# cfframe/spatial-VAE

Hardware: AMD Instinct MI355X
Metric: images/sec (ELBO fwd+bwd+step), MNIST 28x28 batch=256, 1/2/4/8 GPU (higher is better)
Workload: dtype f32; 1 GPU; mnist-rotated-translated 28x28 z=2 H=500x2 tanh B=256 (BASELINE configs[1]); global_batch=256, per_gpu_batch=256, pixels=784, parallelism=dp1

## Files before the change

spatial_vae_amd/csrc/dense.h:

```cpp
#pragma once
#include "common.h"

namespace svae {

struct DenseArgs {
    const float* in;
    const float* wp;
    float* out;
    const float* bias;
    const float* aux;
    long tiles;
    int Hp;
    int H;
    int act;
    int resid;
    PoseArgs pose;
    const float4* posebuf;
    const float* tab;
    float* sgtile;
    float* dfpart;
    long Mp;
    int N, Timg;
    const float* do_p;
    const float* out_w;
// ... 605 lines not shown
#pragma unroll
        for (int t = 0; t < 4; ++t) {
            xa[t] = *reinterpret_cast<const float4*>(sl + t * 256);
            xb[t] = *reinterpret_cast<const float4*>(sl + (4 + t) * 256);
        }
        d = *reinterpret_cast<const float4*>(ring + ((o - o0) & 3) * kSlotFloats + 8 * 256 + h * 4);
    };
    auto frag_post = [&](long o, float4 (&xa)[4], const float4& d) {
        if (own_out) {
            const float wgt = (o < o1) ? 1.0f : 0.0f;
            pbias[0] += wgt * ((d.x + d.y) + (d.z + d.w));
#pragma unroll
            for (int t = 0; t < 4; ++t) pw[0][t] += wgt * ((d.x * xa[t].x + d.y * xa[t].y) + (d.z * xa[t].z + d.w * xa[t].w));
        }
#pragma unroll
        for (int t = 0; t < 4; ++t) {
            const float4 v = xa[t];
            const float4 tt = make_float4(d.x * v.x, d.y * v.y, d.z * v.z, d.w * v.w);
            xa[t] = make_float4(__builtin_fmaf(-tt.x, v.x, R1 == 1 ? d.x : tt.x), __builtin_fmaf(-tt.y, v.y, R1 == 1 ? d.y : tt.y),
                                __builtin_fmaf(-tt.z, v.z, R1 == 1 ? d.z : tt.z), __builtin_fmaf(-tt.w, v.w, R1 == 1 ? d.w : tt.w));
        }
    };
    auto mul = [&](const float4 (&xa)[4], const float4 (&xb)[4]) {
#pragma unroll
        for (int i = 0; i < 4; ++i)
#pragma unroll
            for (int j = 0; j < 4; ++j) acc[i][j] = __builtin_amdgcn_mfma_f32_32x32x2f32(xa[i].x, xb[j].x, acc[i][j], 0, 0, 0);
#pragma unroll
        for (int i = 0; i < 4; ++i)
#pragma unroll
            for (int j = 0; j < 4; ++j) acc[i][j] = __builtin_amdgcn_mfma_f32_32x32x2f32(xa[i].y, xb[j].y, acc[i][j], 0, 0, 0);
#pragma unroll
        for (int i = 0; i < 4; ++i)
#pragma unroll
            for (int j = 0; j < 4; ++j) acc[i][j] = __builtin_amdgcn_mfma_f32_32x32x2f32(xa[i].z, xb[j].z, acc[i][j], 0, 0, 0);
#pragma unroll
        for (int i = 0; i < 4; ++i)
#pragma unroll
            for (int j = 0; j < 4; ++j) acc[i][j] = __builtin_amdgcn_mfma_f32_32x32x2f32(xa[i].w, xb[j].w, acc[i][j], 0, 0, 0);
        if (own_bias) {
#pragma unroll
            for (int t = 0; t < 4; ++t) bs[t] += (xa[t].x + xa[t].y) + (xa[t].z + xa[t].w);
        }
    };
    if (o0 < o1) {
        float4 ca[4], cb[4], na[4], nb[4];
        dma(o0);
        dma(o0 + 1);
        dma(o0 + 2);
        if (CL > 0) asm volatile("s_waitcnt vmcnt(18)" ::: "memory");
        else asm volatile("s_waitcnt vmcnt(16)" ::: "memory");
        float4 nd = make_float4(0.f, 0.f, 0.f, 0.f);
        if (R1 != 0) {
            frag_raw(o0, ca, cb, nd);
            frag_post(o0, ca, nd);
        } else {
            frag(o0, ca, cb);
        }
        for (long o = o0; o < o1; ++o) {
            dma(o + 3);
            if (CL > 0) asm volatile("s_waitcnt vmcnt(18)" ::: "memory");
            else asm volatile("s_waitcnt vmcnt(16)" ::: "memory");
            if (R1 != 0) frag_raw(o + 1, na, nb, nd);
            else frag(o + 1, na, nb);
            if (CL == 0 || R1 != 0) __builtin_amdgcn_sched_barrier(0);
            mul(ca, cb);
            if (CL == 0 || R1 != 0) __builtin_amdgcn_sched_barrier(0);
            if (R1 != 0) frag_post(o + 1, na, nd);
#pragma unroll
            for (int t = 0; t < 4; ++t) {
                ca[t] = na[t];
                cb[t] = nb[t];
            }
        }
        dma_wait_all();
    }

    float* slab = a.slab + (long)split * Hp * Hp;
#pragma unroll
    for (int i = 0; i < 4; ++i) {
        if (ibase + i >= ntile) continue;
#pragma unroll
        for (int j = 0; j < 4; ++j) {
            if (jbase + j >= ntile) continue;
            const int k = (jbase + j) * 32 + nl;
#pragma unroll
            for (int r = 0; r < 16; ++r) {
                const int n = (ibase + i) * 32 + (r & 3) + 8 * (r >> 2) + 4 * h;
                slab[(long)n * Hp + k] = acc[i][j][r];
            }
        }
    }
    if (own_out) {
#pragma unroll
        for (int c = 0; c < CL; ++c) {
#pragma unroll
            for (int i = 0; i < 4; ++i)
                if (ibase + i < ntile) a.wpart[(((long)split * 2 + h) * CL + c) * Hp + (ibase + i) * 32 + nl] = pw[c][i];
            if (bi == 0 && wave == 0 && nl == 0) a.bpart[((long)split * 2 + h) * CL + c] = pbias[c];
        }
    }
    if (own_bias) {
#pragma unroll
        for (int i = 0; i < 4; ++i)
            if (ibase + i < ntile) a.bslab[((long)split * 2 + h) * Hp + (ibase + i) * 32 + nl] = bs[i];
    }
}

struct WgradReduceArgs {
    const float* slab;
    const float* bslab;
    float* dW;
    float* db;
    int H, Hp, S;
    const float* row_scale;
};
__device__ __forceinline__ void wgrad_reduce_block(const WgradReduceArgs& a, unsigned bx, float (*red)[64]) {
    const float* __restrict__ slab = a.slab;
    const float* __restrict__ bslab = a.bslab;
    float* __restrict__ dW = a.dW;
    float* __restrict__ db = a.db;
    const float* __restrict__ row_scale = a.row_scale;
    const int H = a.H, Hp = a.Hp, S = a.S;
    const int col = threadIdx.x & 63, grp = threadIdx.x >> 6;
    const long idx = (long)bx * 64 + col;
    const bool in = idx < (long)H * H;
    float part = 0.0f;
    if (in) {
        const int n = (int)(idx / H), k = (int)(idx - (long)n * H);
        const float* p = slab + (long)n * Hp + k;
        const long st = (long)Hp * Hp;
        float s0 = 0.0f, s1 = 0.0f, s2 = 0.0f, s3 = 0.0f;
        int i = grp;
        for (; i + 12 < S; i += 16) {
            s0 += p[(long)i * st];
            s1 += p[(long)(i + 4) * st];
            s2 += p[(long)(i + 8) * st];
            s3 += p[(long)(i + 12) * st];
        }
        for (; i < S; i += 4) s0 += p[(long)i * st];
        part = (s0 + s1) + (s2 + s3);
    }
    red[grp][col] = part;
    __syncthreads();
    if (grp == 0 && in && dW) {
        const float t = (red[0][col] + red[1][col]) + (red[2][col] + red[3][col]);
        dW[idx] = row_scale ? t * row_scale[idx / H] : t;
    }
    if (db && bx * 64 < (unsigned)H) {
        __syncthreads();
        const int n = bx * 64 + col;
        float s = 0.0f;
        if (n < H)
            for (int i = grp; i < 2 * S; i += 4) s += bslab[(long)i * Hp + n];
        red[grp][col] = s;
        __syncthreads();
        if (grp == 0 && n < H) {
            const float t = (red[0][col] + red[1][col]) + (red[2][col] + red[3][col]);
            db[n] = row_scale ? t * row_scale[n] : t;
        }
    }
}
__global__ void __launch_bounds__(256) wgrad_reduce_kernel(WgradReduceArgs a) {
    __shared__ float red[4][64];
    wgrad_reduce_block(a, blockIdx.x, red);
}

}
```

spatial_vae_amd/csrc/elementwise.h:

```cpp
#pragma once
#include <type_traits>
#include "common.h"

namespace svae {

__device__ __forceinline__ long slab_index(int contr, int out, int ntile) {
    return (((long)(contr >> 3) * ntile + (out >> 5)) * 2 + ((contr >> 2) & 1)) * 128 + (out & 31) * 4 + (contr & 3);
}
struct PrepareArgs {
    const float* coord_w; const float* coord_b; const float* latent_w; const float* bil_w; const float* z;
    float* tab; float4* posebuf; PoseArgs pose;
    int B, H, Hp, Zd, in_dim;
    int nb_tab, nb_pack, nlayers;
    const float* W[SVAE_MAX_HIDDEN]; float* wf[SVAE_MAX_HIDDEN]; float* wb[SVAE_MAX_HIDDEN];
    const float* wb_row_scale[SVAE_MAX_HIDDEN];
};
__global__ void __launch_bounds__(256) prepare_kernel(PrepareArgs a) {
    if ((int)blockIdx.x < a.nb_tab) {
        const long idx = (long)blockIdx.x * 256 + threadIdx.x;
        if (idx < a.B) {
            float c, s, d0, d1;
            image_pose(a.pose, (int)idx, c, s, d0, d1);
            a.posebuf[idx] = make_float4(c, s, d0, d1);
        }
        if (idx >= (long)a.B * a.Hp) return;
        const int b = idx / a.Hp, k = idx % a.Hp;
        float out[kSlots] = {0, 0, 0, 0, 0, 0, 0, 0};
        if (k < a.H) {
            for (int p = 0; p < a.in_dim; ++p) {
                float w = a.coord_w[k * a.in_dim + p];
                if (a.bil_w)
                    for (int q = 0; q < a.Zd; ++q) w += a.bil_w[((long)k * a.in_dim + p) * a.Zd + q] * a.z[(long)b * a.Zd + q];
                out[p] = w;
            }
            float bias = a.coord_b[k];
            if (a.latent_w)
                for (int q = 0; q < a.Zd; ++q) bias += a.latent_w[(long)k * a.Zd + q] * a.z[(long)b * a.Zd + q];
            out[kBiasSlot] = bias;
        }
        float4* dst = reinterpret_cast<float4*>(a.tab + idx * kSlots);
        dst[0] = make_float4(out[0], out[1], out[2], out[3]);
        dst[1] = make_float4(out[4], out[5], out[6], out[7]);
        return;
    }
    const int rel = blockIdx.x - a.nb_tab;
    const int l = rel / a.nb_pack;
    const long idx = (long)(rel - l * a.nb_pack) * 256 + threadIdx.x;
    if (l >= a.nlayers || idx >= (long)a.Hp * a.Hp) return;
    const int n = idx / a.Hp, k = idx % a.Hp;
    const float v = (n < a.H && k < a.H) ? a.W[l][(long)n * a.H + k] : 0.0f;
    a.wf[l][slab_index(k, n, a.Hp / 32)] = v;
    a.wb[l][slab_index(n, k, a.Hp / 32)] = (a.wb_row_scale[l] && n < a.H) ? v * a.wb_row_scale[l][n] : v;
}

struct RowGeo {
    int N, Npad, Hp, in_dim, act, B;
};

constexpr int kL0Chunk = 32;
template <int ACT>
__global__ void __launch_bounds__(256) layer0_fwd_kernel(PoseArgs pose, const float4* __restrict__ posebuf,
                                                         const float* __restrict__ tab, float* __restrict__ a0, RowGeo g,
                                                         int oct_per_chunk, int chunks_per_image, long nchunks) {
    __shared__ float4 xs[kL0Chunk * 2 * 2];
    const long chunk = (long)blockIdx.z * gridDim.y + blockIdx.y;
    if (chunk >= nchunks) return;
    const int b = (int)(chunk / chunks_per_image), ci = (int)(chunk - (long)b * chunks_per_image);
    const int oimg = g.Npad >> 3;
    const int oc0 = ci * oct_per_chunk;
    const int noc = (oc0 + oct_per_chunk <= oimg) ? oct_per_chunk : oimg - oc0;
    const float4 pb = posebuf[b];
    const float* cbase = pose.coords ? pose.coords + (long)b * g.N * 2 : pose.grid;
    float* xf = reinterpret_cast<float*>(xs);
    for (int j = threadIdx.x; j < noc * 8; j += 256) {
        const int i = oc0 * 8 + j;
        float x0 = 0.0f, x1 = 0.0f;
        if (i < g.N) {
            const float2 raw = *reinterpret_cast<const float2*>(cbase + (long)i * 2);
            x0 = pb.x * raw.x - pb.y * raw.y + pb.z;
            x1 = pb.y * raw.x + pb.x * raw.y + pb.w;
        }
        const int slot = (j >> 2) * 8 + (j & 3);
        xf[slot] = x0;
        xf[slot + 4] = x1;
    }
    __syncthreads();
    const int t = blockIdx.x * 256 + threadIdx.x;
    if (t >= g.Hp * 2) return;
    const int h = t & 1, k = t >> 1;
    const float4* tp = reinterpret_cast<const float4*>(tab + ((long)b * g.Hp + k) * kSlots);
    const float4 t0 = tp[0], t1 = tp[1];
    const long ostride = (long)g.Hp * 8;
    float* dst = a0 + (((long)b * oimg + oc0) * g.Hp * 2 + t) * 4;
    const bool expand = g.in_dim == 5;
#pragma unroll 4
    for (int jo = 0; jo < noc; ++jo) {
        const float4 X0 = xs[(jo * 2 + h) * 2], X1 = xs[(jo * 2 + h) * 2 + 1];
        const float x0[4] = {X0.x, X0.y, X0.z, X0.w}, x1[4] = {X1.x, X1.y, X1.z, X1.w};
        float out[4];
#pragma unroll
        for (int e = 0; e < 4; ++e) {
            float v = t1.y + x0[e] * t0.x + x1[e] * t0.y;
            if (expand) v += (x0[e] * x0[e]) * t0.z + (x1[e] * x1[e]) * t0.w + (x0[e] * x1[e]) * t1.x;
            out[e] = act_fwd<ACT>(v);
        }
        *reinterpret_cast<float4*>(dst + jo * ostride) = make_float4(out[0], out[1], out[2], out[3]);
    }
}

template <int C>
__global__ void out_fwd_kernel(const float* __restrict__ a, const float* __restrict__ out_w,
                               const float* __restrict__ out_b, float* __restrict__ y, float* __restrict__ logits,
                               RowGeo g, int H, int softplus, long noct) {
    const int lane = threadIdx.x & 63;
    const int nl = lane & 31, h = lane >> 5;
    const long wave0 = (long)blockIdx.x * 4 + (threadIdx.x >> 6);
    const long nwaves = (long)gridDim.x * 4;
    for (long o = wave0; o < noct; o += nwaves) {
        float p[4][C];
#pragma unroll
        for (int e = 0; e < 4; ++e)
#pragma unroll
            for (int c = 0; c < C; ++c) p[e][c] = 0.0f;
        for (int t = 0; t < g.Hp / 32; ++t) {
            const int n = t * 32 + nl;
            const float4 v = *reinterpret_cast<const float4*>(a + ((o * g.Hp + n) * 8 + 4 * h));
#pragma unroll
            for (int c = 0; c < C; ++c) {
                const float w = (n < H) ? out_w[c * H + n] : 0.0f;
                p[0][c] += v.x * w; p[1][c] += v.y * w; p[2][c] += v.z * w; p[3][c] += v.w * w;
            }
        }
#pragma unroll
        for (int e = 0; e < 4; ++e)
#pragma unroll
            for (int c = 0; c < C; ++c) p[e][c] = wave_sum32(p[e][c]);
        if (nl < 4) {
            const long m = 8 * o + 4 * h + nl;
            const int b = m / g.Npad, i = m % g.Npad;
            if (i < g.N) {
#pragma unroll
                for (int c = 0; c < C; ++c) {
                    const float s0 = nl == 0 ? p[0][c] : nl == 1 ? p[1][c] : nl == 2 ? p[2][c] : p[3][c];
                    const float lg = s0 + out_b[c];
                    float s = 1.0f / (1.0f + expf(-lg));
                    if (softplus && c == 0) s = log1pf(expf(s));
                    const long oi = ((long)b * g.N + i) * C + c;
                    y[oi] = s;
                    if (logits) logits[oi] = lg;
                }
            }
        }
    }
}

__global__ void logits_finish_kernel(const float* __restrict__ lpart, const float* __restrict__ out_b, float* __restrict__ y,
                                     float* __restrict__ logits, RowGeo g, int C, int nblk, int softplus, long Mp, long m_split,
                                     int nblk_tail) {
    const long t = (long)blockIdx.x * 256 + threadIdx.x;
    if (t >= (long)g.B * g.N) return;
    const int b = (int)(t / g.N), i = (int)(t - (long)b * g.N);
    const long m = (long)b * g.Npad + i;
    if (m >= m_split) nblk = nblk_tail;
    for (int c = 0; c < C; ++c) {
        float lg = 0.0f;
        for (int k = 0; k < nblk; ++k) lg += lpart[((long)k * C + c) * Mp + m];
        lg += out_b[c];
        float s = 1.0f / (1.0f + expf(-lg));
        if (softplus && c == 0) s = log1pf(expf(s));
        y[t * C + c] = s;
        if (logits) logits[t * C + c] = lg;
    }
}

__global__ void __launch_bounds__(1024) logits_finish_bce_kernel(const float* __restrict__ lpart, const float* __restrict__ out_b,
                                                                const float* __restrict__ target, float* __restrict__ y,
                                                                float* __restrict__ logits, float* __restrict__ loglik,
                                                                float* __restrict__ dll, RowGeo g, int C, int nblk, long Mp,
                                                                long m_split, int nblk_tail) {
    __shared__ float red[16];
    const int b = blockIdx.x;
    float acc = 0.0f;
    const int per = (g.N + gridDim.y - 1) / gridDim.y;
    const int i0 = blockIdx.y * per, i1 = (i0 + per < g.N) ? i0 + per : g.N;
    for (int i = i0 + threadIdx.x; i < i1; i += blockDim.x) {
        const long m = (long)b * g.Npad + i;
        const long t = (long)b * g.N + i;
        const int nbk = m >= m_split ? nblk_tail : nblk;
        for (int c = 0; c < C; ++c) {
            float lg = 0.0f;
            for (int k = 0; k < nbk; ++k) lg += lpart[((long)k * C + c) * Mp + m];
            lg += out_b[c];
            const float s = 1.0f / (1.0f + expf(-lg));
            const float tg = target[t * C + c];
            y[t * C + c] = s;
            if (logits) logits[t * C + c] = lg;
            const float ls = fmaxf(logf(s), -100.0f);
            const float l1s = fmaxf(log1pf(-s), -100.0f);
            acc += tg * ls + (1.0f - tg) * l1s;
            if (dll) dll[t * C + c] = -(s - tg) / fmaxf((1.0f - s) * s, 1e-12f);
        }
    }
    acc = block_sum_waves(acc, red);
    if (threadIdx.x == 0) loglik[(long)b * gridDim.y + blockIdx.y] = acc;
}

__global__ void loglik_reduce_kernel(const float* __restrict__ part, float* __restrict__ loglik, int B, int chunks) {
    const int b = blockIdx.x * 256 + threadIdx.x;
    if (b >= B) return;
    float s = 0.0f;
    for (int k = 0; k < chunks; ++k) s += part[(long)b * chunks + k];
    loglik[b] = s;
}

__global__ void dlogits_kernel(const float* __restrict__ logits, const float* __restrict__ dy,
                               const float* __restrict__ dy_scale, float* __restrict__ do_p, int B, int N, int Npad,
                               int C, int softplus, long Mp, unsigned* __restrict__ amax) {
    const long idx = (long)blockIdx.x * 256 + threadIdx.x;
    float m = 0.0f;
    if (idx < (long)C * Mp) {
        const int c = (int)(idx / Mp);
        const long mp = idx - (long)c * Mp;
        const int b = (int)(mp / Npad), i = (int)(mp - (long)b * Npad);
        float v = 0.0f;
        if (i < N) {
            const long src = ((long)b * N + i) * C + c;
            const float lg = logits[src];
            const float s = 1.0f / (1.0f + expf(-lg));
            float g = dy[src];
            if (dy_scale) g *= dy_scale[b];
            if (softplus && c == 0) g *= 1.0f / (1.0f + expf(-s));
            v = g * s * (1.0f - s);
        }
        do_p[idx] = v;
        m = fabsf(v);
    }
    if (amax) {
        __shared__ float red[4];
#pragma unroll
        for (int d = 32; d >= 1; d >>= 1) m = fmaxf(m, __shfl_xor(m, d));
        if ((threadIdx.x & 63) == 0) red[threadIdx.x >> 6] = m;
        __syncthreads();
        if (threadIdx.x == 0) {
            m = fmaxf(fmaxf(red[0], red[1]), fmaxf(red[2], red[3]));
            if (m > 0.0f) atomicMax(amax, __float_as_uint(m));
        }
    }
}

template <int ACT, int C>
__global__ void out_bwd_kernel(const float* __restrict__ a, const float* __restrict__ do_p,
                               const float* __restrict__ out_w, float* __restrict__ dh, float* __restrict__ wpart,
                               float* __restrict__ bpart, int H, int Hp, long Mp, long noct, long oct_per_chunk) {
    const int t = blockIdx.x * 256 + threadIdx.x;
    if (t >= Hp * 2) return;
    const int h = t & 1, n = t >> 1;
    float w[C], pw[C], pb[C];
#pragma unroll
    for (int c = 0; c < C; ++c) {
        w[c] = (n < H) ? out_w[c * H + n] : 0.0f;
        pw[c] = 0.0f;
        pb[c] = 0.0f;
    }
    const long o0 = blockIdx.y * oct_per_chunk;
    const long o1 = (o0 + oct_per_chunk < noct) ? o0 + oct_per_chunk : noct;
    for (long o = o0; o < o1; ++o) {
        const long off = (o * Hp + n) * 8 + 4 * h;
        const float4 av = *reinterpret_cast<const float4*>(a + off);
        float4 da = make_float4(0.f, 0.f, 0.f, 0.f);
#pragma unroll
        for (int c = 0; c < C; ++c) {
            const float4 d = *reinterpret_cast<const float4*>(do_p + (long)c * Mp + 8 * o + 4 * h);
            da.x += d.x * w[c]; da.y += d.y * w[c]; da.z += d.z * w[c]; da.w += d.w * w[c];
            pw[c] += (d.x * av.x + d.y * av.y) + (d.z * av.z + d.w * av.w);
            pb[c] += (d.x + d.y) + (d.z + d.w);
        }
        da.x *= act_grad<ACT>(av.x); da.y *= act_grad<ACT>(av.y);
        da.z *= act_grad<ACT>(av.z); da.w *= act_grad<ACT>(av.w);
        *reinterpret_cast<float4*>(dh + off) = da;
    }
#pragma unroll
    for (int c = 0; c < C; ++c) wpart[(((long)blockIdx.y * 2 + h) * C + c) * Hp + n] = pw[c];
    if (n == 0) {
#pragma unroll
        for (int c = 0; c < C; ++c) bpart[((long)blockIdx.y * 2 + h) * C + c] = pb[c];
    }
}

constexpr int kObrLanes = 16;
struct OutBwdReduceArgs {
    const float* wpart;
    const float* bpart;
    float* dWo;
    float* dbo;
    int C, H, Hp, nparts;
};
template <int LPT>
__device__ __forceinline__ void out_bwd_reduce_block(const OutBwdReduceArgs& a, unsigned bx, float (*red)[65]) {
    static_assert(kObrLanes % LPT == 0, "whole part lanes per thread");
    constexpr int LSTEP = kObrLanes / LPT;
    const float* __restrict__ wpart = a.wpart;
    const float* __restrict__ bpart = a.bpart;
    const int C = a.C, H = a.H, Hp = a.Hp, nparts = a.nparts;
    const int col = threadIdx.x & 63, pl0 = threadIdx.x >> 6;
    const int blocks_per_c = (Hp + 63) / 64;
    if (bx == (unsigned)(C * blocks_per_c)) {
#pragma unroll
        for (int l = 0; l < LPT; ++l) {
            const int pl = pl0 + LSTEP * l;
            float s = 0.0f;
            if (col < C)
                for (int i = pl; i < nparts; i += kObrLanes) s += bpart[(long)i * C + col];
            red[pl][col] = s;
        }
        __syncthreads();
        if (pl0 == 0 && col < C && a.dbo) {
            float t = red[0][col];
#pragma unroll
            for (int j = 1; j < kObrLanes; ++j) t += red[j][col];
            a.dbo[col] = t;
        }
        return;
    }
    const int c = bx / blocks_per_c, n = (bx % blocks_per_c) * 64 + col;
    float s[LPT];
#pragma unroll
    for (int l = 0; l < LPT; ++l) s[l] = 0.0f;
    if (n < Hp) {
        const float* p = wpart + (long)c * Hp + n;
        const long st = (long)C * Hp;
        float ch[LPT][8];
        int i[LPT];
#pragma unroll
        for (int l = 0; l < LPT; ++l) {
            i[l] = pl0 + LSTEP * l;
#pragma unroll
            for (int j = 0; j < 8; ++j) ch[l][j] = 0.0f;
        }
        for (bool any = true; any;) {
            any = false;
#pragma unroll
            for (int l = 0; l < LPT; ++l)
                if (i[l] + 7 * kObrLanes < nparts) {
#pragma unroll
                    for (int j = 0; j < 8; ++j) ch[l][j] += p[(long)(i[l] + j * kObrLanes) * st];
                    i[l] += 8 * kObrLanes;
                    any = true;
                }
        }
#pragma unroll
        for (int l = 0; l < LPT; ++l) {
            for (; i[l] < nparts; i[l] += kObrLanes) ch[l][0] += p[(long)i[l] * st];
            s[l] = ((ch[l][0] + ch[l][1]) + (ch[l][2] + ch[l][3])) + ((ch[l][4] + ch[l][5]) + (ch[l][6] + ch[l][7]));
        }
    }
#pragma unroll
    for (int l = 0; l < LPT; ++l) red[pl0 + LSTEP * l][col] = s[l];
    __syncthreads();
    if (pl0 == 0 && n < H && a.dWo) {
        float t = red[0][col];
#pragma unroll
        for (int j = 1; j < kObrLanes; ++j) t += red[j][col];
        a.dWo[(long)c * H + n] = t;
    }
}
__global__ void __launch_bounds__(1024) out_bwd_reduce_kernel(const float* __restrict__ wpart, const float* __restrict__ bpart,
                                                              float* __restrict__ dWo, float* __restrict__ dbo, int C, int H,
                                                              int Hp, int nparts) {
    __shared__ float red[kObrLanes][65];
    out_bwd_reduce_block<1>(OutBwdReduceArgs{wpart, bpart, dWo, dbo, C, H, Hp, nparts}, blockIdx.x, red);
}

__global__ void layer0_bwd_params_kernel(PoseArgs pose, const float4* __restrict__ posebuf,
                                         const float* __restrict__ dh0, float* __restrict__ sgpart, RowGeo g,
                                         int oct_per_chunk, int chunks_per_image) {
    const int t = blockIdx.x * 256 + threadIdx.x;
    if (t >= g.Hp * 2) return;
    const int h = t & 1, k = t >> 1;
    const int b = blockIdx.y / chunks_per_image, ci = blockIdx.y % chunks_per_image;
    const int oimg = g.Npad / 8;
    const int oc0 = ci * oct_per_chunk;
    const int oc1 = (oc0 + oct_per_chunk < oimg) ? oc0 + oct_per_chunk : oimg;
    const float4 pb = posebuf[b];
    float G[5] = {0, 0, 0, 0, 0};
    float S = 0.0f;
    for (int oc = oc0; oc < oc1; ++oc) {
        const long o = (long)b * oimg + oc;
        const float4 d = *reinterpret_cast<const float4*>(dh0 + (o * g.Hp + k) * 8 + 4 * h);
        const float dv[4] = {d.x, d.y, d.z, d.w};
        const int i0 = oc * 8 + 4 * h;
#pragma unroll
        for (int e = 0; e < 4; ++e) {
            const float2 x = row_coord(pose, pb, b, i0 + e, g.N);
            S += dv[e];
            G[0] += dv[e] * x.x;
            G[1] += dv[e] * x.y;
            if (g.in_dim == 5) {
                G[2] += dv[e] * x.x * x.x;
                G[3] += dv[e] * x.y * x.y;
                G[4] += dv[e] * x.x * x.y;
            }
        }
    }
    float4* dst = reinterpret_cast<float4*>(sgpart + (((long)blockIdx.y * g.Hp + k) * 2 + h) * kSlots);
    dst[0] = make_float4(G[0], G[1], G[2], G[3]);
    dst[1] = make_float4(G[4], S, 0.0f, 0.0f);
}

__global__ void sg_reduce_kernel(const float* __restrict__ sgpart, float* __restrict__ sgimg, int B, int Hp,
                                 int chunks_per_image) {
    const long idx = (long)blockIdx.x * 256 + threadIdx.x;
    if (idx >= (long)B * Hp * kSlots) return;
    const int slot = idx % kSlots;
    const long bk = idx / kSlots;
    const int k = bk % Hp, b = bk / Hp;
    float s = 0.0f;
    for (int ci = 0; ci < chunks_per_image; ++ci)
        for (int h = 0; h < 2; ++h)
            s += sgpart[((((long)b * chunks_per_image + ci) * Hp + k) * 2 + h) * kSlots + slot];
    sgimg[idx] = s;
}

__global__ void layer0_bwd_coords_kernel(PoseArgs pose, const float4* __restrict__ posebuf,
                                         const float* __restrict__ dh0, const float* __restrict__ tab,
                                         float* __restrict__ dcoords, RowGeo g, long noct) {
    const int lane = threadIdx.x & 63;
    const int ml = lane & 7, kq = lane >> 3;
    const long wave0 = (long)blockIdx.x * 4 + (threadIdx.x >> 6);
    const long nwaves = (long)gridDim.x * 4;
    for (long o = wave0; o < noct; o += nwaves) {
        const long m = 8 * o + ml;
        const int b = m / g.Npad, i = m % g.Npad;
        float acc[5] = {0, 0, 0, 0, 0};
        for (int k = kq; k < g.Hp; k += 8) {
            const float d = dh0[(o * g.Hp + k) * 8 + ml];
            const float4* tp = reinterpret_cast<const float4*>(tab + ((long)b * g.Hp + k) * kSlots);
            const float4 t0 = tp[0];
            acc[0] += d * t0.x;
            acc[1] += d * t0.y;
            if (g.in_dim == 5) {
                const float4 t1 = tp[1];
                acc[2] += d * t0.z;
                acc[3] += d * t0.w;
                acc[4] += d * t1.x;
            }
        }
#pragma unroll
        for (int p = 0; p < 5; ++p) {
            acc[p] += __shfl_xor(acc[p], 8);
            acc[p] += __shfl_xor(acc[p], 16);
            acc[p] += __shfl_xor(acc[p], 32);
        }
        if (kq == 0 && i < g.N) {
            float d0 = acc[0], d1 = acc[1];
            if (g.in_dim == 5) {
                const float2 x = row_coord(pose, posebuf[b], b, i, g.N);
                d0 += 2.0f * x.x * acc[2] + x.y * acc[4];
                d1 += 2.0f * x.y * acc[3] + x.x * acc[4];
            }
            *reinterpret_cast<float2*>(dcoords + ((long)b * g.N + i) * 2) = make_float2(d0, d1);
        }
    }
}

struct FirstLayerImageArgs {
    const float* sgtile;
    int nhalf, Timg, H, Hp;
    float* sgimg;
    const float* latent_w;
    const float* bil_w;
    float* dz;
    int Zd, in_dim;
    const float* dfpart;
    int nblocks, N, Npad;
    long Mp;
    float* dcoords;
    const float* grid;
    const float4* posebuf;
    float* dtheta;
    float* ddx;
    long m_split;
    int nblocks_tail;
    const float* tab;
};
__device__ __forceinline__ void first_layer_image_block(const FirstLayerImageArgs& a, int b, int role, float* red) {
    const float* __restrict__ sgtile = a.sgtile;
    const int nhalf = a.nhalf, Timg = a.Timg, H = a.H, Hp = a.Hp;
    float* __restrict__ sgimg = a.sgimg;
    const float* __restrict__ latent_w = a.latent_w;
    const float* __restrict__ bil_w = a.bil_w;
    float* __restrict__ dz = a.dz;
    const int Zd = a.Zd, in_dim = a.in_dim;
    const float* __restrict__ dfpart = a.dfpart;
    const int nblocks = a.nblocks, N = a.N, Npad = a.Npad;
    const long Mp = a.Mp;
    float* __restrict__ dcoords = a.dcoords;
    const float* __restrict__ grid = a.grid;
    const float4* __restrict__ posebuf = a.posebuf;
    float* __restrict__ dtheta = a.dtheta;
    float* __restrict__ ddx = a.ddx;
    const long m_split = a.m_split;
    const int nblocks_tail = a.nblocks_tail;

    if (role == 0) {
        const bool pose_sums = a.tab && (dtheta || ddx);
        double pt = 0.0, p0 = 0.0, p1 = 0.0;
        float4 pb = make_float4(1.0f, 0.0f, 0.0f, 0.0f);
        if (pose_sums) pb = posebuf[b];
        for (int k = threadIdx.x; k < Hp; k += 256) {
            const float* src = sgtile + ((long)b * Timg * nhalf * Hp + k) * 4;
            const long rst = (long)Hp * 4;
            const int rows = Timg * nhalf;
            float c0[8] = {0, 0, 0, 0, 0, 0, 0, 0}, c1[8] = {0, 0, 0, 0, 0, 0, 0, 0}, c2[8] = {0, 0, 0, 0, 0, 0, 0, 0};
            double d0 = 0.0, d1 = 0.0, d2 = 0.0;
            int r = 0;
            for (; r + 7 < rows; r += 8) {
#pragma unroll
                for (int j = 0; j < 8; ++j) {
                    const float4 v = *reinterpret_cast<const float4*>(src + (r + j) * rst);
                    c0[j] += v.x; c1[j] += v.y; c2[j] += v.z;
                    if (pose_sums) { d0 += (double)v.x; d1 += (double)v.y; d2 += (double)v.z; }
                }
            }
            for (int j = 0; r < rows; ++r, ++j) {
                const float4 v = *reinterpret_cast<const float4*>(src + r * rst);
                c0[j] += v.x; c1[j] += v.y; c2[j] += v.z;
                if (pose_sums) { d0 += (double)v.x; d1 += (double)v.y; d2 += (double)v.z; }
            }
            if (pose_sums && k < H) {
                const float2 w = *reinterpret_cast<const float2*>(a.tab + ((long)b * Hp + k) * kSlots);
                p0 += (double)w.x * d2;
                p1 += (double)w.y * d2;
                pt += (double)w.y * (d0 - (double)pb.z * d2) - (double)w.x * (d1 - (double)pb.w * d2);
            }
            const float g0 = ((c0[0] + c0[1]) + (c0[2] + c0[3])) + ((c0[4] + c0[5]) + (c0[6] + c0[7]));
            const float g1 = ((c1[0] + c1[1]) + (c1[2] + c1[3])) + ((c1[4] + c1[5]) + (c1[6] + c1[7]));
            const float sv = ((c2[0] + c2[1]) + (c2[2] + c2[3])) + ((c2[4] + c2[5]) + (c2[6] + c2[7]));
            float4* dst = reinterpret_cast<float4*>(sgimg + ((long)b * Hp + k) * kSlots);
            dst[0] = make_float4(g0, g1, 0.0f, 0.0f);
            dst[1] = make_float4(0.0f, sv, 0.0f, 0.0f);
        }
        if (pose_sums) {
            double* redd = reinterpret_cast<double*>(red);
            pt = block_sum256d(pt, redd);
            p0 = block_sum256d(p0, redd);
            p1 = block_sum256d(p1, redd);
            if (threadIdx.x == 0) {
                if (dtheta) dtheta[b] = (float)pt;
                if (ddx) {
                    ddx[2 * b] = (float)p0;
                    ddx[2 * b + 1] = (float)p1;
                }
            }
        }
        if (!dz || Zd <= 0) return;
        for (int q = 0; q < Zd; ++q) {
            float s = 0.0f;
            for (int k = threadIdx.x; k < H; k += 256) {
                const float* e = sgimg + ((long)b * Hp + k) * kSlots;
                s += e[kBiasSlot] * latent_w[(long)k * Zd + q];
                if (bil_w)
                    for (int p = 0; p < in_dim; ++p) s += e[p] * bil_w[((long)k * in_dim + p) * Zd + q];
            }
            s = block_sum256(s, red);
            if (threadIdx.x == 0) dz[(long)b * Zd + q] = s;
        }
        return;
    }
    if (!dcoords) return;
    const bool want_pose = dtheta || ddx;
    float4 pb = make_float4(1.0f, 0.0f, 0.0f, 0.0f);
    if (want_pose) pb = posebuf[b];
    float st = 0.0f, s0 = 0.0f, s1 = 0.0f;
    for (int i = threadIdx.x; i < N; i += 256) {
        const long mp = (long)b * Npad + i;
        float d0 = 0.0f, d1 = 0.0f;
        const int nbk = mp >= m_split ? nblocks_tail : nblocks;
        for (int nb = 0; nb < nbk; ++nb) {
            const float2 v = *reinterpret_cast<const float2*>(dfpart + ((long)nb * Mp + mp) * 2);
            d0 += v.x; d1 += v.y;
        }
        *reinterpret_cast<float2*>(dcoords + ((long)b * N + i) * 2) = make_float2(d0, d1);
        if (want_pose) {
            const float2 gr = *reinterpret_cast<const float2*>(grid + (long)i * 2);
            st += d0 * (-pb.y * gr.x - pb.x * gr.y) + d1 * (pb.x * gr.x - pb.y * gr.y);
            s0 += d0;
            s1 += d1;
        }
    }
    if (!want_pose) return;
    st = block_sum256(st, red);
    s0 = block_sum256(s0, red);
    s1 = block_sum256(s1, red);
    if (threadIdx.x == 0) {
        if (dtheta) dtheta[b] = st;
        if (ddx) {
            ddx[2 * b] = s0;
            ddx[2 * b + 1] = s1;
        }
    }
}

__global__ void __launch_bounds__(256) first_layer_image_kernel(FirstLayerImageArgs a) {
    __shared__ __attribute__((aligned(8))) float red[8];
    first_layer_image_block(a, blockIdx.x, blockIdx.y, red);
}
__global__ void __launch_bounds__(256) backward_tail_kernel(FirstLayerImageArgs f, WgradReduceArgs r, OutBwdReduceArgs o,
                                                            unsigned nimg, unsigned nred, int B) {
    __shared__ __attribute__((aligned(8))) float red[kObrLanes * 65];
    if (blockIdx.x < nimg) first_layer_image_block(f, (int)(blockIdx.x % (unsigned)B), (int)(blockIdx.x / (unsigned)B), red);
    else if (blockIdx.x < nimg + nred) wgrad_reduce_block(r, blockIdx.x - nimg, reinterpret_cast<float (*)[64]>(red));
    else out_bwd_reduce_block<4>(o, blockIdx.x - nimg - nred, reinterpret_cast<float (*)[65]>(red));
}

constexpr int kZChunk = 8;
constexpr int kPgCols = 16, kPgLanes = 16;
__global__ void __launch_bounds__(256) layer0_param_grads_kernel(const float* __restrict__ sgimg, const float* __restrict__ z,
                                                                 float* __restrict__ dWc, float* __restrict__ dbc,
                                                                 float* __restrict__ dWz, float* __restrict__ dWbi, int B, int H,
                                                                 int Hp, int Zd, int in_dim) {
    __shared__ float red[kPgLanes][kPgCols + 1];
    const int col = threadIdx.x & (kPgCols - 1), bl = threadIdx.x / kPgCols;
    const int t = blockIdx.x * kPgCols + col;
    const bool in_range = t < H * kSlots;
    const int k = in_range ? t / kSlots : 0, slot = in_range ? t % kSlots : 0;
    const bool is_g = in_range && slot < in_dim, is_s = in_range && slot == kBiasSlot;
    const float* src = sgimg + (long)k * kSlots + slot;
    const long bstride = (long)Hp * kSlots;
    auto combine = [&](float v) {
        __syncthreads();
        red[bl][col] = v;
        __syncthreads();
        float r = red[0][col];
#pragma unroll
        for (int j = 1; j < kPgLanes; ++j) r += red[j][col];
        return r;
    };
    const bool want_z = (is_s && dWz) || (is_g && dWbi);
    const int nq0 = Zd < kZChunk ? Zd : kZChunk;
    float plain = 0.0f;
    float acc[kZChunk];
#pragma unroll
    for (int q = 0; q < kZChunk; ++q) acc[q] = 0.0f;
    if (is_g || is_s) {
        int b = bl;
        for (; b + 3 * kPgLanes < B; b += 4 * kPgLanes) {
            float v[4];
#pragma unroll
            for (int j = 0; j < 4; ++j) v[j] = src[(long)(b + j * kPgLanes) * bstride];
#pragma unroll
            for (int j = 0; j < 4; ++j) {
                plain += v[j];
                if (want_z) {
#pragma unroll
                    for (int q = 0; q < kZChunk; ++q)
                        if (q < nq0) acc[q] += v[j] * z[(long)(b + j * kPgLanes) * Zd + q];
                }
            }
        }
        for (; b < B; b += kPgLanes) {
            const float v = src[(long)b * bstride];
            plain += v;
            if (want_z) {
#pragma unroll
                for (int q = 0; q < kZChunk; ++q)
                    if (q < nq0) acc[q] += v * z[(long)b * Zd + q];
            }
        }
    }
    plain = combine(plain);
    if (bl == 0) {
        if (is_g && dWc) dWc[k * in_dim + slot] = plain;
        if (is_s && dbc) dbc[k] = plain;
    }
    for (int q0 = 0; q0 < Zd; q0 += kZChunk) {
        if (q0 > 0) {
#pragma unroll
            for (int q = 0; q < kZChunk; ++q) acc[q] = 0.0f;
            if (want_z)
                for (int b = bl; b < B; b += kPgLanes) {
                    const float v = src[(long)b * bstride];
#pragma unroll
                    for (int q = 0; q < kZChunk; ++q)
                        if (q0 + q < Zd) acc[q] += v * z[(long)b * Zd + q0 + q];
                }
        }
#pragma unroll
        for (int q = 0; q < kZChunk; ++q) {
            if (q0 + q >= Zd) break;
            const float r = combine(acc[q]);
            if (bl == 0 && want_z) {
                if (is_s) dWz[(long)k * Zd + q0 + q] = r;
                else dWbi[((long)k * in_dim + slot) * Zd + q0 + q] = r;
            }
        }
    }
}

__global__ void dz_kernel(const float* __restrict__ sgimg, const float* __restrict__ latent_w,
                          const float* __restrict__ bil_w, float* __restrict__ dz, int H, int Hp, int Zd, int in_dim) {
    __shared__ float red[4];
    const int b = blockIdx.x;
    for (int q = 0; q < Zd; ++q) {
        float s = 0.0f;
        for (int k = threadIdx.x; k < H; k += 256) {
            const float* e = sgimg + ((long)b * Hp + k) * kSlots;
            s += e[kBiasSlot] * latent_w[(long)k * Zd + q];
            if (bil_w)
                for (int p = 0; p < in_dim; ++p) s += e[p] * bil_w[((long)k * in_dim + p) * Zd + q];
        }
        s = block_sum256(s, red);
        if (threadIdx.x == 0) dz[(long)b * Zd + q] = s;
    }
}

__global__ void pose_bwd_kernel(const float* __restrict__ dcoords, const float* __restrict__ grid,
                                const float4* __restrict__ posebuf, float* __restrict__ dtheta,
                                float* __restrict__ ddx, int N) {
    __shared__ float red[4];
    const int b = blockIdx.x;
    const float4 pb = posebuf[b];
    float st = 0.0f, s0 = 0.0f, s1 = 0.0f;
    for (int i = threadIdx.x; i < N; i += 256) {
        const float2 d = *reinterpret_cast<const float2*>(dcoords + ((long)b * N + i) * 2);
        const float2 gr = *reinterpret_cast<const float2*>(grid + (long)i * 2);
        st += d.x * (-pb.y * gr.x - pb.x * gr.y) + d.y * (pb.x * gr.x - pb.y * gr.y);
        s0 += d.x;
        s1 += d.y;
    }
    st = block_sum256(st, red);
    s0 = block_sum256(s0, red);
    s1 = block_sum256(s1, red);
    if (threadIdx.x == 0) {
        if (dtheta) dtheta[b] = st;
        if (ddx) {
            ddx[2 * b] = s0;
            ddx[2 * b + 1] = s1;
        }
    }
}

__global__ void bce_kernel(const float* __restrict__ y_hat, const float* __restrict__ target,
                           float* __restrict__ loglik, float* __restrict__ dll, int n) {
    __shared__ float red[4];
    const int b = blockIdx.x;
    float acc = 0.0f;
    for (int j = threadIdx.x; j < n; j += 256) {
        const long idx = (long)b * n + j;
        const float s = y_hat[idx], t = target[idx];
        const float ls = fmaxf(logf(s), -100.0f);
        const float l1s = fmaxf(log1pf(-s), -100.0f);
        acc += t * ls + (1.0f - t) * l1s;
        if (dll) dll[idx] = -(s - t) / fmaxf((1.0f - s) * s, 1e-12f);
    }
    acc = block_sum256(acc, red);
    if (threadIdx.x == 0) loglik[b] = acc;
}

__global__ void gaussian_kernel(const float* __restrict__ yp, const float* __restrict__ target,
                                const uint8_t* __restrict__ mask, const float* __restrict__ ctf, int k,
                                float* __restrict__ loglik, float* __restrict__ dll, float* __restrict__ filt,
                                float* __restrict__ dflt, int N, int C) {
    __shared__ float red[4];
    const int b = blockIdx.x;
    const int n = (int)(sqrtf((float)N) + 0.5f);
    const float* row = yp + (long)b * N * C;
    const bool noise = C > 1;
    const int pad = k / 2;
// ... 679 lines not shown
```

spatial_vae_amd/csrc/encoder.h:

```cpp
#pragma once
#include "common.h"

namespace svae {

constexpr int SVAE_ACT_NONE = -1;

__device__ __forceinline__ float enc_act(int act, float v) {
    switch (act) {
        case SVAE_ACT_TANH: return fast_tanh(v);
        case SVAE_ACT_LEAKYRELU: return v > 0.0f ? v : 0.01f * v;
        case SVAE_ACT_RELU: return v > 0.0f ? v : 0.0f;
        case SVAE_ACT_SIGMOID: return fast_sigmoid(v);
        default: return v;
    }
}
__device__ __forceinline__ float enc_act_grad(int act, float a) {
    switch (act) {
        case SVAE_ACT_TANH: return 1.0f - a * a;
        case SVAE_ACT_LEAKYRELU: return a > 0.0f ? 1.0f : 0.01f;
        case SVAE_ACT_RELU: return a > 0.0f ? 1.0f : 0.0f;
        case SVAE_ACT_SIGMOID: return a * (1.0f - a);
        default: return 1.0f;
    }
}

struct LinFwdArgs {
    const float* x;
    const float* w;
    const float* b;
    float* out;
    int M, K, N, act;
};

constexpr int kEncUnroll = 16;

__device__ __forceinline__ void enc_reduce4(v4f& acc, float& extra, float (*red)[5][64]) {
    const int lane = threadIdx.x & 63, wave = threadIdx.x >> 6;
#pragma unroll
    for (int r = 0; r < 4; ++r) red[wave][r][lane] = acc[r];
    red[wave][4][lane] = extra;
    __syncthreads();
    if (wave == 0) {
#pragma unroll
        for (int r = 0; r < 4; ++r) acc[r] = (red[0][r][lane] + red[1][r][lane]) + (red[2][r][lane] + red[3][r][lane]);
        extra = (red[0][4][lane] + red[1][4][lane]) + (red[2][4][lane] + red[3][4][lane]);
    }
}

template <bool VEC>
__global__ void __launch_bounds__(256) enc_linear_fwd_kernel(LinFwdArgs a) {
    __shared__ float red[4][5][64];
    const int lane = threadIdx.x & 63, i = lane & 15, g = lane >> 4, wave = threadIdx.x >> 6;
    const int tiles_n = (a.N + 15) >> 4;
    const int tm = blockIdx.x / tiles_n, tn = blockIdx.x - tm * tiles_n;
    const int row = tm * 16 + i, col = tn * 16 + i;
    const bool va = row < a.M, vb = col < a.N;
    const float* ap = a.x + (long)(va ? row : a.M - 1) * a.K;
    const float* bp = a.w + (long)(vb ? col : a.N - 1) * a.K;
    v4f acc = {0.0f, 0.0f, 0.0f, 0.0f};
    if (VEC) {
        const int groups = (a.K + 15) >> 4;
        const int per = (groups + 3) >> 2;
        const int u0 = wave * per, u1 = (u0 + per < groups) ? u0 + per : groups;
        constexpr int U = kEncUnroll / 2;
        for (int ub = u0; ub < u1; ub += U) {
            float4 av[U], bv[U];
#pragma unroll
            for (int u = 0; u < U; ++u) {
                const int k = (ub + u) * 16 + 4 * g;
                const bool in = ub + u < u1 && k < a.K;
                const int kc = in ? k : 0;
                av[u] = *reinterpret_cast<const float4*>(ap + kc);
                bv[u] = *reinterpret_cast<const float4*>(bp + kc);
                if (!in || !va) av[u] = make_float4(0.f, 0.f, 0.f, 0.f);
                if (!in || !vb) bv[u] = make_float4(0.f, 0.f, 0.f, 0.f);
            }
#pragma unroll
            for (int u = 0; u < U; ++u) {
                acc = __builtin_amdgcn_mfma_f32_16x16x4f32(av[u].x, bv[u].x, acc, 0, 0, 0);
                acc = __builtin_amdgcn_mfma_f32_16x16x4f32(av[u].y, bv[u].y, acc, 0, 0, 0);
                acc = __builtin_amdgcn_mfma_f32_16x16x4f32(av[u].z, bv[u].z, acc, 0, 0, 0);
                acc = __builtin_amdgcn_mfma_f32_16x16x4f32(av[u].w, bv[u].w, acc, 0, 0, 0);
            }
        }
    } else {
        const int steps = (a.K + 3) >> 2;
        const int per = (steps + 3) >> 2;
        const int s0 = wave * per, s1 = (s0 + per < steps) ? s0 + per : steps;
        for (int sb = s0; sb < s1; sb += kEncUnroll) {
            float av[kEncUnroll], bv[kEncUnroll];
#pragma unroll
            for (int u = 0; u < kEncUnroll; ++u) {
                const int k = (sb + u) * 4 + g;
                const bool in = sb + u < s1 && k < a.K;
                const int kc = in ? k : 0;
                av[u] = (in && va) ? ap[kc] : 0.0f;
                bv[u] = (in && vb) ? bp[kc] : 0.0f;
            }
#pragma unroll
            for (int u = 0; u < kEncUnroll; ++u) acc = __builtin_amdgcn_mfma_f32_16x16x4f32(av[u], bv[u], acc, 0, 0, 0);
        }
    }
    float none = 0.0f;
    enc_reduce4(acc, none, red);
    if (wave != 0) return;
    const int n = tn * 16 + i;
    if (n < a.N) {
        const float bias = a.b ? a.b[n] : 0.0f;
#pragma unroll
        for (int r = 0; r < 4; ++r) {
            const int m = tm * 16 + 4 * g + r;
            if (m < a.M) a.out[(long)m * a.N + n] = enc_act(a.act, acc[r] + bias);
        }
    }
}

struct LinBwdArgs {
    const float* x;
    const float* w;
    const float* out;
    const float* dout;
    float* dw;
    float* db;
    float* dx;
    int M, K, N, act;
    int tiles_w;
};

template <bool VECX>
__global__ void __launch_bounds__(256) enc_linear_bwd_kernel(LinBwdArgs a) {
    __shared__ float red[4][5][64];
    const int lane = threadIdx.x & 63, i = lane & 15, g = lane >> 4, wave = threadIdx.x >> 6;
    const int tiles_k = (a.K + 15) >> 4;
    const bool has_act = a.act != SVAE_ACT_NONE;
    v4f acc = {0.0f, 0.0f, 0.0f, 0.0f};
    float bsum = 0.0f;
    if ((int)blockIdx.x < a.tiles_w) {
        const int tn = blockIdx.x / tiles_k, tk = blockIdx.x - tn * tiles_k;
        const int n = tn * 16 + i, k = tk * 16 + i;
        const bool vn = n < a.N, vk = k < a.K;
        const int nc = vn ? n : a.N - 1, kc = vk ? k : a.K - 1;
        const int steps = (a.M + 3) >> 2;
        const int per = (steps + 3) >> 2;
        const int s0 = wave * per, s1 = (s0 + per < steps) ? s0 + per : steps;
        for (int sb = s0; sb < s1; sb += kEncUnroll) {
            float dv[kEncUnroll], ov[kEncUnroll], xv[kEncUnroll];
#pragma unroll
            for (int u = 0; u < kEncUnroll; ++u) {
                const long m = (long)(sb + u) * 4 + g;
                const bool in = sb + u < s1 && m < a.M;
                const long mc = in ? m : 0;
                dv[u] = (in && vn) ? a.dout[mc * a.N + nc] : 0.0f;
                ov[u] = has_act ? a.out[mc * a.N + nc] : 0.0f;
                xv[u] = (in && vk) ? a.x[mc * a.K + kc] : 0.0f;
            }
#pragma unroll
            for (int u = 0; u < kEncUnroll; ++u) {
                const float dp = dv[u] * enc_act_grad(a.act, ov[u]);
                bsum += dp;
                acc = __builtin_amdgcn_mfma_f32_16x16x4f32(dp, xv[u], acc, 0, 0, 0);
            }
        }
        enc_reduce4(acc, bsum, red);
        if (wave != 0) return;
        if (a.dw && vk) {
#pragma unroll
            for (int r = 0; r < 4; ++r) {
                const int nn = tn * 16 + 4 * g + r;
                if (nn < a.N) a.dw[(long)nn * a.K + k] = acc[r];
            }
        }
        if (tk == 0 && a.db) {
            bsum += __shfl_xor(bsum, 32);
            bsum += __shfl_xor(bsum, 16);
            if (g == 0 && vn) a.db[n] = bsum;
        }
        return;
    }
    if (!a.dx) return;
    const int t = blockIdx.x - a.tiles_w;
    const int tm = t / tiles_k, tk = t - tm * tiles_k;
    const int row = tm * 16 + i, k = tk * 16 + i;
    const bool vr = row < a.M, vk = k < a.K;
    const long rc = vr ? row : a.M - 1;
    const int kc = vk ? k : a.K - 1;
    if (VECX) {
        const int groups = (a.N + 15) >> 4;
        const int per = (groups + 3) >> 2;
        const int u0 = wave * per, u1 = (u0 + per < groups) ? u0 + per : groups;
        constexpr int U = kEncUnroll / 4;
        for (int ub = u0; ub < u1; ub += U) {
            float4 dv[U], ov[U];
            float wv[U][4];
#pragma unroll
            for (int u = 0; u < U; ++u) {
                const int n = (ub + u) * 16 + 4 * g;
                const bool in = ub + u < u1 && n < a.N;
                const int ncl = in ? n : 0;
                dv[u] = *reinterpret_cast<const float4*>(a.dout + rc * a.N + ncl);
                ov[u] = has_act ? *reinterpret_cast<const float4*>(a.out + rc * a.N + ncl) : make_float4(0.f, 0.f, 0.f, 0.f);
                if (!in || !vr) dv[u] = make_float4(0.f, 0.f, 0.f, 0.f);
#pragma unroll
                for (int t = 0; t < 4; ++t) wv[u][t] = (in && vk) ? a.w[(long)(ncl + t) * a.K + kc] : 0.0f;
            }
#pragma unroll
            for (int u = 0; u < U; ++u) {
                acc = __builtin_amdgcn_mfma_f32_16x16x4f32(dv[u].x * enc_act_grad(a.act, ov[u].x), wv[u][0], acc, 0, 0, 0);
                acc = __builtin_amdgcn_mfma_f32_16x16x4f32(dv[u].y * enc_act_grad(a.act, ov[u].y), wv[u][1], acc, 0, 0, 0);
                acc = __builtin_amdgcn_mfma_f32_16x16x4f32(dv[u].z * enc_act_grad(a.act, ov[u].z), wv[u][2], acc, 0, 0, 0);
                acc = __builtin_amdgcn_mfma_f32_16x16x4f32(dv[u].w * enc_act_grad(a.act, ov[u].w), wv[u][3], acc, 0, 0, 0);
            }
        }
    }
    const int steps = VECX ? 0 : (a.N + 3) >> 2;
    const int per = (steps + 3) >> 2;
    const int s0 = wave * per, s1 = (s0 + per < steps) ? s0 + per : steps;
    for (int sb = s0; sb < s1; sb += kEncUnroll) {
        float dv[kEncUnroll], ov[kEncUnroll], wv[kEncUnroll];
// ... 26 lines not shown
```

Baseline: 98780 images/s.

## Batch loads in flight in reductions and fuse first dz chunk into image pass

Several reduction loops (bias grad slab sum, logits partial sum, per-image sgtile row sum) are restructured to issue up to 16 independent loads before accumulating, which raises memory-level parallelism. The first-layer image block now computes the first eight latent dz components inside the same per-k loop and merges the pose and dz reductions into one shuffle pass with a single barrier, instead of running separate block reductions and a second sweep over sgimg. The encoder linear forward gets a single-shot path that loads all K groups at once when each wave holds few of them. The cost is more registers per thread, and the shared reduction buffer grows from 8 to 64 floats.

```diff
diff --git a/spatial_vae_amd/csrc/dense.h b/spatial_vae_amd/csrc/dense.h
--- a/spatial_vae_amd/csrc/dense.h
+++ b/spatial_vae_amd/csrc/dense.h
@@ -781,7 +781,15 @@
         const int n = bx * 64 + col;
         float s = 0.0f;
         if (n < H)
-            for (int i = grp; i < 2 * S; i += 4) s += bslab[(long)i * Hp + n];
+            for (int i0 = grp; i0 < 2 * S; i0 += 64) {
+                float v[16];
+#pragma unroll
+                for (int j = 0; j < 16; ++j)
+                    if (i0 + 4 * j < 2 * S) v[j] = bslab[(long)(i0 + 4 * j) * Hp + n];
+#pragma unroll
+                for (int j = 0; j < 16; ++j)
+                    if (i0 + 4 * j < 2 * S) s += v[j];
+            }
         red[grp][col] = s;
         __syncthreads();
         if (grp == 0 && n < H) {
diff --git a/spatial_vae_amd/csrc/elementwise.h b/spatial_vae_amd/csrc/elementwise.h
--- a/spatial_vae_amd/csrc/elementwise.h
+++ b/spatial_vae_amd/csrc/elementwise.h
@@ -173,6 +173,7 @@
     }
 }
 
+constexpr int kFinishFlight = 16;
 __global__ void __launch_bounds__(1024) logits_finish_bce_kernel(const float* __restrict__ lpart, const float* __restrict__ out_b,
                                                                 const float* __restrict__ target, float* __restrict__ y,
                                                                 float* __restrict__ logits, float* __restrict__ loglik,
@@ -189,7 +190,15 @@
         const int nbk = m >= m_split ? nblk_tail : nblk;
         for (int c = 0; c < C; ++c) {
             float lg = 0.0f;
-            for (int k = 0; k < nbk; ++k) lg += lpart[((long)k * C + c) * Mp + m];
+            for (int k0 = 0; k0 < nbk; k0 += kFinishFlight) {
+                float v[kFinishFlight];
+#pragma unroll
+                for (int k = 0; k < kFinishFlight; ++k)
+                    if (k0 + k < nbk) v[k] = lpart[((long)(k0 + k) * C + c) * Mp + m];
+#pragma unroll
+                for (int k = 0; k < kFinishFlight; ++k)
+                    if (k0 + k < nbk) lg += v[k];
+            }
             lg += out_b[c];
             const float s = 1.0f / (1.0f + expf(-lg));
             const float tg = target[t * C + c];
@@ -483,6 +492,8 @@
     int nblocks_tail;
     const float* tab;
 };
+constexpr int kZChunk = 8;
+constexpr int kImgFlight = 16;
 __device__ __forceinline__ void first_layer_image_block(const FirstLayerImageArgs& a, int b, int role, float* red) {
     const float* __restrict__ sgtile = a.sgtile;
     const int nhalf = a.nhalf, Timg = a.Timg, H = a.H, Hp = a.Hp;
@@ -504,28 +515,31 @@
 
     if (role == 0) {
         const bool pose_sums = a.tab && (dtheta || ddx);
+        const bool want_dz = dz && Zd > 0;
+        const int nq0 = Zd < kZChunk ? Zd : kZChunk;
         double pt = 0.0, p0 = 0.0, p1 = 0.0;
+        float zs[kZChunk];
+#pragma unroll
+        for (int q = 0; q < kZChunk; ++q) zs[q] = 0.0f;
         float4 pb = make_float4(1.0f, 0.0f, 0.0f, 0.0f);
         if (pose_sums) pb = posebuf[b];
+        const long rst = (long)Hp * 4;
+        const int rows = Timg * nhalf;
         for (int k = threadIdx.x; k < Hp; k += 256) {
-            const float* src = sgtile + ((long)b * Timg * nhalf * Hp + k) * 4;
-            const long rst = (long)Hp * 4;
-            const int rows = Timg * nhalf;
+            const float* src = sgtile + ((long)b * rows * Hp + k) * 4;
             float c0[8] = {0, 0, 0, 0, 0, 0, 0, 0}, c1[8] = {0, 0, 0, 0, 0, 0, 0, 0}, c2[8] = {0, 0, 0, 0, 0, 0, 0, 0};
             double d0 = 0.0, d1 = 0.0, d2 = 0.0;
-            int r = 0;
-            for (; r + 7 < rows; r += 8) {
-#pragma unroll
-                for (int j = 0; j < 8; ++j) {
-                    const float4 v = *reinterpret_cast<const float4*>(src + (r + j) * rst);
-                    c0[j] += v.x; c1[j] += v.y; c2[j] += v.z;
-                    if (pose_sums) { d0 += (double)v.x; d1 += (double)v.y; d2 += (double)v.z; }
-                }
-            }
-            for (int j = 0; r < rows; ++r, ++j) {
-                const float4 v = *reinterpret_cast<const float4*>(src + r * rst);
-                c0[j] += v.x; c1[j] += v.y; c2[j] += v.z;
-                if (pose_sums) { d0 += (double)v.x; d1 += (double)v.y; d2 += (double)v.z; }
+            for (int rb = 0; rb < rows; rb += kImgFlight) {
+                float4 v[kImgFlight];
+#pragma unroll
+                for (int j = 0; j < kImgFlight; ++j)
+                    if (rb + j < rows) v[j] = *reinterpret_cast<const float4*>(src + (rb + j) * rst);
+#pragma unroll
+                for (int j = 0; j < kImgFlight; ++j)
+                    if (rb + j < rows) {
+                        c0[j & 7] += v[j].x; c1[j & 7] += v[j].y; c2[j & 7] += v[j].z;
+                        if (pose_sums) { d0 += (double)v[j].x; d1 += (double)v[j].y; d2 += (double)v[j].z; }
+                    }
             }
             if (pose_sums && k < H) {
                 const float2 w = *reinterpret_cast<const float2*>(a.tab + ((long)b * Hp + k) * kSlots);
@@ -539,22 +553,56 @@
             float4* dst = reinterpret_cast<float4*>(sgimg + ((long)b * Hp + k) * kSlots);
             dst[0] = make_float4(g0, g1, 0.0f, 0.0f);
             dst[1] = make_float4(0.0f, sv, 0.0f, 0.0f);
-        }
+            if (want_dz && k < H) {
+                const float e[5] = {g0, g1, 0.0f, 0.0f, 0.0f};
+#pragma unroll
+                for (int q = 0; q < kZChunk; ++q)
+                    if (q < nq0) {
+                        zs[q] += sv * latent_w[(long)k * Zd + q];
+                        if (bil_w) {
+#pragma unroll
+                            for (int p = 0; p < 5; ++p)
+                                if (p < in_dim) zs[q] += e[p] * bil_w[((long)k * in_dim + p) * Zd + q];
+                        }
+                    }
+            }
+        }
+        if (!pose_sums && !want_dz) return;
+        double* redd = reinterpret_cast<double*>(red);
+        float* redf = red + 24;
+        const int lane = threadIdx.x & 63, wave = threadIdx.x >> 6;
         if (pose_sums) {
-            double* redd = reinterpret_cast<double*>(red);
-            pt = block_sum256d(pt, redd);
-            p0 = block_sum256d(p0, redd);
-            p1 = block_sum256d(p1, redd);
-            if (threadIdx.x == 0) {
-                if (dtheta) dtheta[b] = (float)pt;
+#pragma unroll
+            for (int m = 1; m < 64; m <<= 1) {
+                pt += __shfl_xor(pt, m);
+                p0 += __shfl_xor(p0, m);
+                p1 += __shfl_xor(p1, m);
+            }
+            if (lane == 0) { redd[wave] = pt; redd[4 + wave] = p0; redd[8 + wave] = p1; }
+        }
+        if (want_dz) {
+#pragma unroll
+            for (int q = 0; q < kZChunk; ++q)
+                if (q < nq0) {
+                    float s = wave_sum32(zs[q]);
+                    s += __shfl_xor(s, 32);
+                    if (lane == 0) redf[q * 4 + wave] = s;
+                }
+        }
+        __syncthreads();
+        if (threadIdx.x == 0) {
+            if (pose_sums) {
+                if (dtheta) dtheta[b] = (float)((redd[0] + redd[1]) + (redd[2] + redd[3]));
                 if (ddx) {
-                    ddx[2 * b] = (float)p0;
-                    ddx[2 * b + 1] = (float)p1;
+                    ddx[2 * b] = (float)((redd[4] + redd[5]) + (redd[6] + redd[7]));
+                    ddx[2 * b + 1] = (float)((redd[8] + redd[9]) + (redd[10] + redd[11]));
                 }
             }
-        }
-        if (!dz || Zd <= 0) return;
-        for (int q = 0; q < Zd; ++q) {
+            if (want_dz)
+                for (int q = 0; q < nq0; ++q) dz[(long)b * Zd + q] = redf[q * 4] + redf[q * 4 + 1] + redf[q * 4 + 2] + redf[q * 4 + 3];
+        }
+        if (!want_dz) return;
+        for (int q = kZChunk; q < Zd; ++q) {
             float s = 0.0f;
             for (int k = threadIdx.x; k < H; k += 256) {
                 const float* e = sgimg + ((long)b * Hp + k) * kSlots;
@@ -602,7 +650,7 @@
 }
 
 __global__ void __launch_bounds__(256) first_layer_image_kernel(FirstLayerImageArgs a) {
-    __shared__ __attribute__((aligned(8))) float red[8];
+    __shared__ __attribute__((aligned(8))) float red[64];
     first_layer_image_block(a, blockIdx.x, blockIdx.y, red);
 }
 __global__ void __launch_bounds__(256) backward_tail_kernel(FirstLayerImageArgs f, WgradReduceArgs r, OutBwdReduceArgs o,
@@ -613,7 +661,6 @@
     else out_bwd_reduce_block<4>(o, blockIdx.x - nimg - nred, reinterpret_cast<float (*)[65]>(red));
 }
 
-constexpr int kZChunk = 8;
 constexpr int kPgCols = 16, kPgLanes = 16;
 __global__ void __launch_bounds__(256) layer0_param_grads_kernel(const float* __restrict__ sgimg, const float* __restrict__ z,
                                                                  float* __restrict__ dWc, float* __restrict__ dbc,
diff --git a/spatial_vae_amd/csrc/encoder.h b/spatial_vae_amd/csrc/encoder.h
--- a/spatial_vae_amd/csrc/encoder.h
+++ b/spatial_vae_amd/csrc/encoder.h
@@ -62,8 +62,31 @@
         const int groups = (a.K + 15) >> 4;
         const int per = (groups + 3) >> 2;
         const int u0 = wave * per, u1 = (u0 + per < groups) ? u0 + per : groups;
+        const int cnt = __builtin_amdgcn_readfirstlane(u1 - u0);
+        if (cnt <= kEncUnroll) {
+            float4 av[kEncUnroll], bv[kEncUnroll];
+#pragma unroll
+            for (int u = 0; u < kEncUnroll; ++u)
+                if (u < cnt) {
+                    const int k = (u0 + u) * 16 + 4 * g;
+                    const bool in = k < a.K;
+                    const int kc = in ? k : 0;
+                    av[u] = *reinterpret_cast<const float4*>(ap + kc);
+                    bv[u] = *reinterpret_cast<const float4*>(bp + kc);
+                    if (!in || !va) av[u] = make_float4(0.f, 0.f, 0.f, 0.f);
+                    if (!in || !vb) bv[u] = make_float4(0.f, 0.f, 0.f, 0.f);
+                }
+#pragma unroll
+            for (int u = 0; u < kEncUnroll; ++u)
+                if (u < cnt) {
+                    acc = __builtin_amdgcn_mfma_f32_16x16x4f32(av[u].x, bv[u].x, acc, 0, 0, 0);
+                    acc = __builtin_amdgcn_mfma_f32_16x16x4f32(av[u].y, bv[u].y, acc, 0, 0, 0);
+                    acc = __builtin_amdgcn_mfma_f32_16x16x4f32(av[u].z, bv[u].z, acc, 0, 0, 0);
+                    acc = __builtin_amdgcn_mfma_f32_16x16x4f32(av[u].w, bv[u].w, acc, 0, 0, 0);
+                }
+        }
         constexpr int U = kEncUnroll / 2;
-        for (int ub = u0; ub < u1; ub += U) {
+        for (int ub = cnt <= kEncUnroll ? u1 : u0; ub < u1; ub += U) {
             float4 av[U], bv[U];
 #pragma unroll
             for (int u = 0; u < U; ++u) {
```

After: 98700 images/s. About the same (-0.1%).
